# HKUST-Aerial-Robotics/D2SLAM

Measured on AMD Instinct MI355X. Metric: frames/sec SuperPoint+NetVLAD+match, 640x480 stereo, higher is better.
Workload: dtype f32

## Files before the change

### d2slam_amd/api.py

```python
import ctypes as C
import os
from dataclasses import dataclass, field
from typing import List, Optional

import numpy as np

from .weights import SP_LAYERS

_HERE = os.path.dirname(os.path.abspath(__file__))
LIB_PATH = os.path.join(_HERE, "lib", "libd2fe_hip.so")
DEV_LIB_PATH = os.path.join(_HERE, "lib", "libd2fe_hip_dev.so")
if os.environ.get("D2FE_LIB"):
    LIB_PATH = os.path.abspath(os.environ["D2FE_LIB"])

POSTPROC_B, POSTPROC_A = 0, 1
PREC_F32, PREC_F16X2, PREC_F32_WINO = 0, 1, 2
ERR_TRUNCATED = -4
KEEP_ALL_CAP = 1024
PROF_STAGES = ["conv1a", "conv1b", "conv2a", "conv2b", "conv3a", "conv3b", "conv4a", "conv4b", "convPaDa",
               "convPb", "convDb", "softmax_cand", "select", "sample", "match", "netvlad", "lk"]


class D2FEError(RuntimeError):
    def __init__(self, code, msg):
# ... 186 lines not shown
    "d2fe_quad_pipe_lanes", "d2fe_quad_pipe_geometry", "d2fe_quad_undistort_device",
    "d2fe_quad_device_view", "d2fe_quad_device_release", "d2fe_quad_lane_stream", "d2fe_quad_handle",
    "d2fe_quad_exchange_default_config", "d2fe_quad_exchange_create", "d2fe_quad_exchange_destroy", "d2fe_quad_exchange_enqueue", "d2fe_quad_exchange_collect",
    "d2fe_quad_exchange_jobs", "d2fe_quad_exchange_pairs", "d2fe_quad_exchange_block_bytes", "d2fe_quad_exchange_stream", "d2fe_quad_exchange_gathered", "d2fe_quad_exchange_job_layout",
    "d2fe_exchange_default_config", "d2fe_exchange_create", "d2fe_exchange_destroy", "d2fe_exchange_enqueue", "d2fe_exchange_collect", "d2fe_exchange_pairs",
    "d2fe_exchange_block_bytes", "d2fe_exchange_stream", "d2fe_exchange_gathered",
    "d2fe_window_default_config", "d2fe_window_create", "d2fe_window_create_quad", "d2fe_window_destroy", "d2fe_window_stream", "d2fe_window_push",
    "d2fe_window_push_host", "d2fe_window_retain", "d2fe_window_retain_plan", "d2fe_window_size", "d2fe_window_tags", "d2fe_window_track_device", "d2fe_window_collect",
    "d2fe_loop_default_config", "d2fe_loop_create", "d2fe_loop_create_quad", "d2fe_loop_destroy", "d2fe_loop_enqueue", "d2fe_loop_collect", "d2fe_loop_ntotal",
    "d2fe_loop_keyframes", "d2fe_loop_stream", "d2fe_loop_query_device", "d2fe_loop_add_host", "d2fe_rccl_load", "d2fe_rccl_path", "d2fe_rccl_unique_id", "d2fe_rccl_comm_init_rank", "d2fe_rccl_comm_destroy"]
DEBUG_EXPORTS = [
    "d2fe_debug_graph_count", "d2fe_debug_read", "d2fe_debug_netvlad_layer", "d2fe_debug_netvlad_stamps", "d2fe_debug_pack_wino",
    "d2fe_debug_pack_netvlad", "d2fe_debug_netvlad_tile", "d2fe_debug_conv3x3_wino", "d2fe_debug_match_stamps",
    "d2fe_debug_netvlad_plan", "d2fe_debug_regime_counts", "d2fe_debug_regime_reset"]
REGIMES = ["wino_nt1_one", "wino_nt1_static", "wino_nt1_claimed", "wino_nt2_one", "wino_nt2_static", "wino_nt2_claimed_ring", "wino_nt2_claimed_fused1b",
           "match_nw4", "match_nw2", "nv_gmerge", "nv_front_tpw", "wino_last_grid", "wino_last_total"]


def _preload_hip_runtime():
    import importlib.util
    import sys
    if "torch" in sys.modules:
        return
    try:
        spec = importlib.util.find_spec("torch")
    except (ImportError, ValueError):
        spec = None
    if spec is not None and spec.origin:
        cand = os.path.join(os.path.dirname(spec.origin), "lib", "libamdhip64.so")
        if os.path.exists(cand):
            try:
# ... 1572 lines not shown
```

### d2slam_amd/build.py

```python
import json
import os
import subprocess
import sys
from concurrent.futures import ThreadPoolExecutor

HERE = os.path.dirname(os.path.abspath(__file__))
CSRC = os.path.join(HERE, "csrc")
LIBDIR = os.path.join(HERE, "lib")
LIB = os.path.join(LIBDIR, "libd2fe_hip.so")
SOURCES = ["api.hip", "conv.hip", "conv_f16.hip", "conv_pc.hip", "conv_wino.hip", "conv1x1.hip", "postproc.hip", "match.hip", "netvlad.hip", "netvlad_fused.hip", "netvlad_pair.hip", "netvlad_host.hip", "next.hip", "swarm.hip", "lk.hip", "lk_carry.hip", "pipe.hip", "exchange.hip", "quad_pipe.hip", "quad_exchange.hip", "loop.hip", "window.hip"]
HEADERS = ["kernels.h", "conv_common.h", "context.h", "stream_deal.h", "lk_device.h", "consumer.h", "lane_ring.h", "exchange_wire.h", os.path.join("..", "..", "include", "d2fe.h"), os.path.join("..", "..", "include", "d2fe_debug.h")]
FLAGS = ["--offload-arch=gfx950", "-O3", "-std=c++17", "-fPIC", "-ffp-contract=off", "-fvisibility=hidden",
         "-Wall", "-Wno-unused-function", "-Wno-unused-result", "-Wno-unused-value"]


EXTRA_FLAGS = {"conv_wino.hip": ["-mllvm", "-amdgpu-atomic-optimizer-strategy=None"]}


def _hipcc():
    for c in (os.environ.get("HIPCC"), "/opt/rocm/bin/hipcc", "hipcc"):
        if c and (os.path.isabs(c) and os.path.exists(c) or not os.path.isabs(c)):
            return c
    return "hipcc"


def needs_build(lib=None):
# ... 78 lines not shown
```

### d2slam_amd/csrc/api.hip

```cpp
#include <hip/hip_runtime.h>

#include <algorithm>
#include <cmath>
#include <cstdio>
#include <cstring>
#include <cstdlib>
#include <array>
#include <atomic>
#include <deque>
#include <map>
#include <mutex>
#include <string>
#include <vector>

#include "context.h"
#ifdef D2FE_DEVTOOLS
#include "../../include/d2fe_debug.h"
#endif

using namespace d2fe;

namespace {
thread_local std::string g_err;
}
// ... 81 lines not shown
    return fail(D2FE_ERR_INVALID, std::string("superpoint layer ") + name + ": unexpected shape");
  return D2FE_OK;
}

}

namespace d2fe {
void graphs_clear(d2fe_context* h) {
  if (h->graphs.empty()) return;
  (void)hipStreamSynchronize(h->stream);
  for (auto& kv : h->graphs) if (kv.second.exec) (void)hipGraphExecDestroy(kv.second.exec);
  h->graphs.clear();
}

void host_state_save(const d2fe_context* h, d2fe_context::HostState& st) {
  st.last_w = h->last_w; st.last_h = h->last_h; st.last_n = h->last_n; st.last_set = h->last_set;
  st.last_gray = h->last_gray; st.last_stride = h->last_stride; st.last_istride = h->last_istride;
  st.nv = h->nv_run.last;
}
void host_state_restore(d2fe_context* h, const d2fe_context::HostState& st, bool netvlad) {
  if (netvlad) {
    h->nv_run.last = st.nv;
  } else {
    h->last_w = st.last_w; h->last_h = st.last_h; h->last_n = st.last_n; h->last_set = st.last_set;
    h->last_gray = st.last_gray; h->last_stride = st.last_stride; h->last_istride = st.last_istride;
  }
}

int run_superpoint(d2fe_context* h, const uint8_t* d_gray, int n, int W, int H, int stride, size_t image_stride,
                   float* d_kps, float* d_scores, float* d_desc, int32_t* d_idx, int cap, int32_t* d_n, hipStream_t s,
                   hipStream_t s_tail, int bs) {
  Tensor& a4b = bs ? h->a4b2 : h->a4b;
  Tensor& logits = bs ? h->logits2 : h->logits;
  Tensor& draw = bs ? h->draw2 : h->draw;
  h->last_set = bs;
  const int prec = h->cfg.precision;
  const bool tail_elsewhere = s_tail && s_tail != s;
  const bool wctr = prec == D2FE_PREC_F32_WINO && h->wino_dynamic;
  if (wctr || !tail_elsewhere)
// ... 7 lines not shown
    a.cout_real = L.cout; a.wpack = L.wpack; a.bias = L.bias;
    a.img = d_gray; a.img_stride = stride; a.img_istride = (long)image_stride; a.w1a = h->w1a; a.b1a = h->b1a;
    a.H = hh; a.W = ww; a.n_img = n; a.in_img_stride = iis; a.out_img_stride = ois; a.zeros = h->zeros; a.ncu = h->ncu;
    a.tag = (&L == &h->L[L_1B]) ? 1 : 0;
    a.work_ctr = (prec == D2FE_PREC_F32_WINO && h->wino_dynamic) ? h->work_ctrs + (int)(&L - &h->L[0]) : nullptr;
    { static const int ab = d2fe_dev_env("D2FE_ABLATE", 0); a.ablate = ab; }
    if (prec != D2FE_PREC_F16X2 && shape == CONV_256_1x1_T4x16 && L.cout == 65 && !pool && !relu) {
      static const int on = d2fe_dev_env("D2FE_CONV1X1", 1);
      if (on) { const hipError_t e = launch_conv1x1_256_65(a, s); if (e != hipErrorNotSupported) return e; }
    }
    if (prec == D2FE_PREC_F32_WINO)
      return shape == CONV1B_FUSED ? launch_conv_wino_fused1b(L.cout_pad, a, s)
             : (L.ks == 3 && !direct) ? launch_conv_wino(L.cin, pool, relu, L.cout_pad, a, s) : launch_conv(shape, D2FE_PREC_F32, pool, relu, L.cout_pad, a, s);
    return launch_conv(shape, prec, pool, relu, L.cout_pad, a, s);
  };
  if (h->fuse1a) {
    ProfScope ps(h, D2FE_PROF_CONV1B, s);
    HIP_TRY(conv(CONV1B_FUSED, h->L[L_1B], nullptr, 64, 0, 0, h->a1b.p, 64, (long)H2 * W2 * 64, H, W, true, true));
  } else {
    { ProfScope ps(h, D2FE_PROF_CONV1A, s); HIP_TRY(launch_conv1a(d_gray, stride, (long)image_stride, H, W, n, h->w1a, h->b1a, h->a1a.p, s)); }
    { ProfScope ps(h, D2FE_PROF_CONV1B, s); HIP_TRY(conv(CONV_64_T8x32, h->L[L_1B], h->a1a.p, 64, 0, (long)H * W * 64, h->a1b.p, 64, (long)H2 * W2 * 64, H, W, true, true)); }
  }
  { ProfScope ps(h, D2FE_PROF_CONV2A, s); HIP_TRY(conv(CONV_64_T8x32, h->L[L_2A], h->a1b.p, 64, 0, (long)H2 * W2 * 64, h->a2a.p, 64, (long)H2 * W2 * 64, H2, W2, false, true)); }
  { ProfScope ps(h, D2FE_PROF_CONV2B, s); HIP_TRY(conv(CONV_64_T8x32, h->L[L_2B], h->a2a.p, 64, 0, (long)H2 * W2 * 64, h->a2b.p, 64, (long)H4 * W4 * 64, H2, W2, true, true)); }
  { ProfScope ps(h, D2FE_PROF_CONV3A, s); HIP_TRY(conv(CONV_64_T8x32, h->L[L_3A], h->a2b.p, 64, 0, (long)H4 * W4 * 64, h->a3a.p, 128, (long)H4 * W4 * 128, H4, W4, false, true)); }
  { ProfScope ps(h, D2FE_PROF_CONV3B, s); HIP_TRY(conv(CONV_128_T4x32, h->L[L_3B], h->a3a.p, 128, 0, (long)H4 * W4 * 128, h->a3b.p, 128, (long)Hc * Wc * 128, H4, W4, true, true)); }
  { ProfScope ps(h, D2FE_PROF_CONV4A, s); HIP_TRY(conv(CONV_128_T4x16, h->L[L_4A], h->a3b.p, 128, 0, (long)Hc * Wc * 128, h->a4a.p, 128, (long)Hc * Wc * 128, Hc, Wc, false, true)); }
  { ProfScope ps(h, D2FE_PROF_CONV4B, s); HIP_TRY(conv(CONV_128_T4x16, h->L[L_4B], h->a4a.p, 128, 0, (long)Hc * Wc * 128, a4b.p, 128, (long)Hc * Wc * 128, Hc, Wc, false, true)); }
  const bool sparse = h->sparse_desc && n >= h->sp_min_batch && 4 * (long)cap <= h->sp_slots;
  if (sparse) {
    { ProfScope ps(h, D2FE_PROF_CONVPADA, s); HIP_TRY(conv(CONV_128_T4x16, h->L[L_PA], a4b.p, 128, 0, (long)Hc * Wc * 128, h->aPD.p, 256, (long)Hc * Wc * 256, Hc, Wc, false, true)); }
    { ProfScope ps(h, D2FE_PROF_CONVPB, s); HIP_TRY(conv(CONV_256_1x1_T4x16, h->L[L_PB], h->aPD.p, 256, 0, (long)Hc * Wc * 256, logits.p, 65, (long)Hc * Wc * 65, Hc, Wc, false, false)); }
  } else {
    if (prec == D2FE_PREC_F32_WINO && h->sparse_desc) {
      ProfScope ps(h, D2FE_PROF_CONVPADA, s);
      HIP_TRY(conv(CONV_128_T4x16, h->L[L_PA], a4b.p, 128, 0, (long)Hc * Wc * 128, h->aPD.p, 512, (long)Hc * Wc * 512, Hc, Wc, false, true));
      HIP_TRY(conv(CONV_128_T4x16, h->L[L_DA32], a4b.p, 128, 0, (long)Hc * Wc * 128, h->aPD.p, 512, (long)Hc * Wc * 512, Hc, Wc, false, true, 256, true));
    } else
    { ProfScope ps(h, D2FE_PROF_CONVPADA, s); HIP_TRY(conv(CONV_128_T4x16, h->L[L_PADA], a4b.p, 128, 0, (long)Hc * Wc * 128, h->aPD.p, 512, (long)Hc * Wc * 512, Hc, Wc, false, true)); }
    { ProfScope ps(h, D2FE_PROF_CONVPB, s); HIP_TRY(conv(CONV_256_1x1_T4x16, h->L[L_PB], h->aPD.p, 512, 0, (long)Hc * Wc * 512, logits.p, 65, (long)Hc * Wc * 65, Hc, Wc, false, false)); }
    { ProfScope ps(h, D2FE_PROF_CONVDB, s); HIP_TRY(conv(CONV_256_1x1_T4x16, h->L[L_DB], h->aPD.p, 512, 256, (long)Hc * Wc * 512, draw.p, 256, (long)Hc * Wc * 256, Hc, Wc, false, false)); }
  }
  const bool varA = h->cfg.postproc == D2FE_POSTPROC_A;
  if (s_tail && s_tail != s) {
    HIP_TRY(hipEventRecord(h->ev_trunk[bs], s));
    HIP_TRY(hipStreamWaitEvent(s_tail, h->ev_trunk[bs], 0));
    s = s_tail;
  }
  { ProfScope ps(h, D2FE_PROF_SOFTMAX, s);
  HIP_TRY(launch_softmax_cand(logits.p, 65, Hc, Wc, n, h->cfg.keypoint_threshold, h->cfg.remove_borders,
                              (h->cfg.keep_score_map || varA || h->cfg.max_keypoints < 0) ? h->semi.p : nullptr,
                              h->cand, h->cand_count, varA ? 0 : h->cand_cap, tail_elsewhere, s)); }
  if (varA) {
    ProfScope ps(h, D2FE_PROF_SELECT, s);
    HIP_TRY(launch_nms2_a(h->semi.p, H, W, n, h->cfg.keypoint_threshold, h->cfg.nms_dist, h->aconf, h->clist, h->cand,
                          h->cand_count, h->cand_cap, h->a_ncand, s));
    HIP_TRY(launch_select_b(h->cand, h->cand_count, h->cand_cap, n, W, h->cfg.max_keypoints < 0 ? h->a_scap : h->cfg.max_keypoints, cap, 1, nullptr, H,
                            h->cfg.keypoint_threshold, 0, d_kps, d_scores, d_idx, d_n, s));
    if ((long)H * W > 65536)
      HIP_TRY(launch_nms2_wrap_fix(h->clist, h->a_ncand, H, W, n, d_kps, d_idx, d_n, cap, s));
  } else {
    ProfScope ps(h, D2FE_PROF_SELECT, s);
    HIP_TRY(launch_select_b(h->cand, h->cand_count, h->cand_cap, n, Wc * 8, h->cfg.max_keypoints, cap, 0,
                            (h->cfg.keep_score_map || h->cfg.max_keypoints < 0) ? h->semi.p : nullptr, Hc * 8, h->cfg.keypoint_threshold,
                            h->cfg.remove_borders, d_kps, d_scores, d_idx, d_n, s));
  }
  if (!sparse) {
// ... 3 lines not shown
                              h->pca_mean, h->pca_dims, h->a_samp, h->a_scap, h->a_cn, nullptr, 0, d_desc, s));
    else
      HIP_TRY(launch_sample_b(draw.p, 256, 0, Hc, Wc, n, d_kps, d_n, cap, nullptr, 0, d_desc, s));
  } else {
    { ProfScope ps(h, D2FE_PROF_CONVDB, s);
      HIP_TRY(launch_desc_head_sparse(d_kps, d_n, cap, Hc, Wc, n, a4b.p, 128, (long)Hc * Wc * 128, h->L[L_DA32].wpack, h->L[L_DA32].bias,
                                      h->L[L_DB32].wpack, h->L[L_DB32].bias, h->sp_flags, h->sp_slotmap, h->sp_cells, h->sp_count,
                                      h->sp_slots, h->sp_desc, h->sp_mid, h->sp_mid_imgs, varA ? W : 0, varA ? H : 0, s)); }
    ProfScope ps(h, D2FE_PROF_SAMPLE, s);
    if (varA)
      HIP_TRY(launch_sample_a(h->sp_desc, 256, 0, Hc, Wc, W, H, n, d_kps, d_n, cap, h->pca_dims ? h->pca_comp_t : nullptr,
                              h->pca_mean, h->pca_dims, h->a_samp, h->a_scap, h->a_cn, h->sp_slotmap, h->sp_slots, d_desc, s));
    else
      HIP_TRY(launch_sample_b(h->sp_desc, 256, 0, Hc, Wc, n, d_kps, d_n, cap, h->sp_slotmap, h->sp_slots, d_desc, s));
  }
  h->last_w = W; h->last_h = H; h->last_n = n;
  h->last_gray = d_gray; h->last_stride = stride; h->last_istride = image_stride;
  return D2FE_OK;
}

int check_geometry(d2fe_context* h, int n, int W, int H, int stride, int cap) {
  if (!h) return fail(D2FE_ERR_INVALID, "null handle");
  if (!h->sp_loaded) return fail(D2FE_ERR_NOT_READY, "superpoint weights not loaded");
  if (n < 1 || n > h->cfg.max_batch) return fail(D2FE_ERR_INVALID, "batch size out of range");
  if (W < 16 || H < 16 || W > h->cfg.max_width || H > h->cfg.max_height || (long)W * H > (long)h->cfg.max_width * h->cfg.max_height)
    return fail(D2FE_ERR_INVALID, "image size must be at least 16x16 and within the configured maximum");
  if (((W | H) & 7) && h->cfg.postproc == D2FE_POSTPROC_A)
    return fail(D2FE_ERR_INVALID, "post-processing variant A needs image sizes that are multiples of 8");
  if (stride < W) return fail(D2FE_ERR_INVALID, "stride < width");
  if (cap < 1) return fail(D2FE_ERR_INVALID, "cap < 1");
  return D2FE_OK;
// ... 50 lines not shown
    int rc = 0;
    if (!h->fuse1a) rc |= alloc_f(h->a1a, H * W * 64, B);
    rc |= alloc_f(h->a1b, H * W * 16, B);
    rc |= alloc_f(h->a2a, H * W * 16, B);
    rc |= alloc_f(h->a2b, H * W * 4, B);
    rc |= alloc_f(h->a3a, H * W * 8, B);
    rc |= alloc_f(h->a3b, H * W * 2, B);
    rc |= alloc_f(h->a4a, H * W * 2, B);
    rc |= alloc_f(h->a4b, H * W * 2, B);
    rc |= alloc_f(h->aPD, H * W * 8, B);
    rc |= alloc_f(h->logits, (H / 8) * (W / 8) * 65, B);
    rc |= alloc_f(h->draw, H * W * 4, B);
    rc |= alloc_f(h->semi, H * W, B);
    if (rc) return D2FE_ERR_HIP;
    h->cand_cap = (long)(H * W);
    HIP_TRY(hipMalloc(&h->cand, sizeof(unsigned long long) * h->cand_cap * B));
    HIP_TRY(hipMalloc(&h->work_ctrs, (64 + ((size_t)B + 63) / 64 * 64) * sizeof(int)));
    HIP_TRY(hipMemset(h->work_ctrs, 0, (64 + ((size_t)B + 63) / 64 * 64) * sizeof(int)));
    h->cand_count = h->work_ctrs + 64;
    if (cfg->async_tail) {
      HIP_TRY(hipStreamCreateWithFlags(&h->tail_stream, hipStreamNonBlocking));
      for (int i = 0; i < 2; ++i) {
        HIP_TRY(hipEventCreateWithFlags(&h->ev_trunk[i], hipEventDisableTiming));
        HIP_TRY(hipEventCreateWithFlags(&h->ev_tail[i], hipEventDisableTiming));
      }
      if (alloc_f(h->a4b2, H * W * 2, B) || alloc_f(h->logits2, (H / 8) * (W / 8) * 65, B) || alloc_f(h->draw2, H * W * 4, B)) return D2FE_ERR_HIP;
    }
    h->sparse_desc = !cfg->dense_descriptors;
    if (cfg->precision == D2FE_PREC_F32_WINO) h->sp_min_batch = 2;
    h->sp_min_batch = d2fe_dev_env("D2FE_SPARSE_MIN_BATCH", h->sp_min_batch);
// ... 891 lines not shown
long d2fe_debug_read(d2fe_handle h, const char* name, void* dst, size_t max_bytes) {
  if (!h || !name || !dst) return fail(D2FE_ERR_INVALID, "null argument");
  if (h->last_n == 0) return fail(D2FE_ERR_NOT_READY, "no extract call yet");
  hipSetDevice(h->cfg.device_id);
  const size_t H = h->last_h, W = h->last_w, n = h->last_n;
  struct { const char* nm; Tensor* t; size_t per; } tab[] = {
      {"conv1a", &h->a1a, H * W * 64},           {"conv1b", &h->a1b, (H / 2) * (W / 2) * 64},   {"conv2a", &h->a2a, (H / 2) * (W / 2) * 64},
      {"conv2b", &h->a2b, (H / 4) * (W / 4) * 64},   {"conv3a", &h->a3a, (H / 4) * (W / 4) * 128},  {"conv3b", &h->a3b, (H / 8) * (W / 8) * 128},
      {"conv4a", &h->a4a, (H / 8) * (W / 8) * 128},  {"conv4b", h->last_set ? &h->a4b2 : &h->a4b, (H / 8) * (W / 8) * 128},  {"convPaDa", &h->aPD, (H / 8) * (W / 8) * 512},
      {"logits", h->last_set ? &h->logits2 : &h->logits, (H / 8) * (W / 8) * 65}, {"desc_raw", h->last_set ? &h->draw2 : &h->draw, (H / 8) * (W / 8) * 256}, {"semi", &h->semi, (H / 8) * (W / 8) * 64}};
  if (!strcmp(name, "conv1a") && h->fuse1a) {
    if (!h->a1a.p && alloc_f(h->a1a, (size_t)h->cfg.max_height * h->cfg.max_width * 64, h->cfg.max_batch) != 0)
      return fail(D2FE_ERR_HIP, "hipMalloc conv1a debug buffer");
    if (launch_conv1a(h->last_gray, h->last_stride, (long)h->last_istride, (int)H, (int)W, (int)n, h->w1a, h->b1a, h->a1a.p, h->stream) != hipSuccess)
      return fail(D2FE_ERR_HIP, "conv1a debug launch");
  }
  if (!strcmp(name, "semi") && !h->cfg.keep_score_map) return fail(D2FE_ERR_NOT_READY, "score map not kept (set keep_score_map)");
  if (h->sparse_desc && h->last_n >= h->sp_min_batch && (!strcmp(name, "desc_raw") || !strcmp(name, "convPaDa")))
    return fail(D2FE_ERR_NOT_READY, "the dense descriptor map does not exist with the sparse descriptor head (set dense_descriptors)");
  for (auto& e : tab)
    if (!strcmp(e.nm, name)) {
      const size_t bytes = e.per * n * sizeof(float);
      if (bytes > max_bytes) return fail(D2FE_ERR_TRUNCATED, "destination too small");
      if (hipStreamSynchronize(h->stream) != hipSuccess || (h->tail_stream && hipStreamSynchronize(h->tail_stream) != hipSuccess)) return fail(D2FE_ERR_HIP, "sync");
      if (hipMemcpy(dst, e.t->p, bytes, hipMemcpyDeviceToHost) != hipSuccess) return fail(D2FE_ERR_HIP, "D2H");
      return (long)bytes;
    }
  return fail(D2FE_ERR_INVALID, "unknown tensor name");
}

// ... 175 lines not shown
```

### d2slam_amd/csrc/context.h

```cpp
#pragma once
#include <hip/hip_runtime.h>

#include <atomic>

#include <array>
#include <deque>
#include <map>
#include <memory>
#include <mutex>
#include <string>
#include <vector>

#include "../../include/d2fe.h"
#include "kernels.h"

namespace d2fe {
int ctx_fail(int code, const std::string& msg);
}

#define HIP_TRY(expr)                                                                                       \
  do {                                                                                                      \
    hipError_t e_ = (expr);                                                                                 \
    if (e_ != hipSuccess)                                                                                   \
      return d2fe::ctx_fail(D2FE_ERR_HIP, std::string(#expr) + ": " + hipGetErrorString(e_) + " @" + __FILE__ + ":" + \
// ... 81 lines not shown
  std::atomic<int> live_pipes{0};
  float* w1a = nullptr;
  float* b1a = nullptr;
  d2fe::Layer L[d2fe::L_COUNT];
  d2fe::Tensor a1a, a1b, a2a, a2b, a3a, a3b, a4a, a4b, aPD, logits, draw, semi;
  d2fe::Tensor a4b2, logits2, draw2;
  hipStream_t tail_stream = nullptr;
  hipEvent_t ev_trunk[2] = {nullptr, nullptr}, ev_tail[2] = {nullptr, nullptr};
  int parity = 0, last_set = 0;
  unsigned long long* cand = nullptr;
  int* cand_count = nullptr;
  long cand_cap = 0;
  uint8_t* s_img = nullptr;
  int s_cap = 0;
  int last_w = 0, last_h = 0, last_n = 0;
  const uint8_t* last_gray = nullptr; int last_stride = 0; size_t last_istride = 0;
  float* aconf = nullptr; int* clist = nullptr; int* a_ncand = nullptr;
  float* zeros = nullptr;
  uint8_t* pin_in = nullptr; size_t pin_in_bytes = 0;
  float* pin_out = nullptr; size_t pin_out_bytes = 0;
  float* s_out = nullptr;
  size_t s_out_bytes = 0;
  bool use_graphs = true, use_pinned = true;
  hipStream_t nv_stream = nullptr; hipEvent_t ev_up = nullptr; float* pin_nv = nullptr; size_t pin_nv_bytes = 0;
  struct HostState { int last_w = 0, last_h = 0, last_n = 0, last_set = 0; const uint8_t* last_gray = nullptr; int last_stride = 0; size_t last_istride = 0;
                     d2fe::NvLast nv; };
  struct GraphEntry { hipGraphExec_t exec = nullptr; int seen = 0; bool bad = false; HostState st; };
  std::map<std::array<long, 6>, GraphEntry> graphs;
  int ncu = 256;
  int ncu_dev = 256;
  unsigned long long* match_stamps = nullptr;
  int32_t* match_stats = nullptr;
  int* work_ctrs = nullptr;
  bool wino_dynamic = true;
  bool sparse_desc = false; int sp_slots = 0; int sp_min_batch = 4;
  uint8_t* sp_flags = nullptr; int32_t* sp_slotmap = nullptr; int32_t* sp_cells = nullptr; int32_t* sp_count = nullptr; float* sp_desc = nullptr;
  float* sp_mid = nullptr; int sp_mid_imgs = 0;
  void* lk_scratch = nullptr; size_t lk_scratch_bytes = 0;
  float* a_samp = nullptr; float* a_cn = nullptr; int a_scap = 0;
  float* pca_comp_t = nullptr; float* pca_mean = nullptr; int pca_dims = 0;
// ... 85 lines not shown
```

### d2slam_amd/csrc/conv1x1.hip

```cpp
#include "conv_common.h"

namespace d2fe {

namespace {
constexpr int C1_CIN = 256, C1_C8 = C1_CIN / 8, C1_RING = 8;
}

__global__ __launch_bounds__(256, 2) void conv1x1_256_65_kernel(ConvArgs a, long npix) {
  extern __shared__ __attribute__((aligned(16))) float wsm[];
  const int tid = threadIdx.x, lane = tid & 63, wave = tid >> 6, hh = lane >> 5;
  const float* wp = reinterpret_cast<const float*>(a.wpack);
  for (int i = tid; i < 2 * C1_C8 * 64; i += 256)
    reinterpret_cast<f32x4*>(wsm)[i] = reinterpret_cast<const f32x4*>(wp)[i];
  float* wdl = wsm + 2 * C1_C8 * 256;
  if (tid < C1_C8 * 8) {
    const int g = tid >> 3, h = (tid >> 2) & 1, q = tid & 3;
    wdl[tid] = wp[((size_t)2 * C1_C8 + g) * 256 + h * 128 + q];
  }
  const float bias0 = a.bias[lane & 31], bias1 = a.bias[32 + (lane & 31)], biasd = a.bias[64];
  __syncthreads();

  const long n_mt = (npix + 31) / 32;
  const int ics = a.in_cstride, ocs = a.out_cstride;
  for (long mt = (long)blockIdx.x * 4 + wave; mt < n_mt; mt += (long)gridDim.x * 4) {
// ... 55 lines not shown
  const long hw = (long)a.H * a.W;
  if (a.cout_real != 65 || a.in_img_stride != hw * a.in_cstride || a.out_img_stride != hw * a.out_cstride || a.out_cstride < 65 ||
      (a.in_cstride & 3) || (a.in_coff & 3) || a.in_coff + 256 > a.in_cstride)
    return hipErrorNotSupported;
  const int ncu = a.ncu > 0 ? a.ncu : 256;
  const long npix = hw * a.n_img;
  const long n_wg = (npix + 127) / 128;
  const int grid = (int)(n_wg < 2 * ncu ? n_wg : 2 * ncu);
  constexpr size_t lds = (size_t)(2 * C1_C8 * 256 + C1_C8 * 8) * sizeof(float);
  hipError_t e = hipFuncSetAttribute(reinterpret_cast<const void*>(conv1x1_256_65_kernel), hipFuncAttributeMaxDynamicSharedMemorySize, (int)lds);
  if (e != hipSuccess) return e;
  hipLaunchKernelGGL(conv1x1_256_65_kernel, dim3(grid), dim3(256), lds, s, a, npix);
  return hipGetLastError();
}

}
```

### d2slam_amd/csrc/kernels.h

```cpp
#pragma once
#include <hip/hip_runtime.h>
#include <stdint.h>

#ifdef D2FE_DEVTOOLS
#include <cstdlib>
static inline int d2fe_dev_env(const char* name, int dflt) { const char* e = getenv(name); return e ? atoi(e) : dflt; }
#define D2FE_ABL(a, bits) ((a).ablate & (bits))
#define D2FE_STAMP(buf, wg, i) do { if ((buf) && threadIdx.x == 0) (buf)[(size_t)(wg) * 16 + (i)] = wall_clock64(); } while (0)
#else
static inline int d2fe_dev_env(const char*, int dflt) { return dflt; }
#define D2FE_ABL(a, bits) (0)
#define D2FE_STAMP(buf, wg, i) do {} while (0)
#endif

#ifdef D2FE_DEVTOOLS
#include "../../include/d2fe_debug.h"
namespace d2fe { void regime_note(int regime); void regime_set(int regime, long long value); }
#define D2FE_REGIME(r) ::d2fe::regime_note(r)
#define D2FE_REGIME_SET(r, v) ::d2fe::regime_set(r, v)
#else
#define D2FE_REGIME(r) do {} while (0)
#define D2FE_REGIME_SET(r, v) do {} while (0)
#endif

// ... 19 lines not shown
  int ncu = 0;
};

enum ConvShape {
  CONV_64_T8x32 = 0,
  CONV_128_T4x32,
  CONV_128_T4x16,
  CONV_256_1x1_T4x16,
  CONV1B_FUSED,
};

hipError_t launch_conv(ConvShape shape, int precision, bool pool, bool relu, int cout_pad, const ConvArgs& a,
                       hipStream_t s);

hipError_t launch_conv1x1_256_65(const ConvArgs& a, hipStream_t s);

hipError_t launch_conv_pc(ConvShape shape, int precision, bool pool, bool relu, int cout_pad, const ConvArgs& a, hipStream_t s);

hipError_t launch_conv_wino(int cin, bool pool, bool relu, int cout_pad, const ConvArgs& a, hipStream_t s);
hipError_t launch_conv_wino_fused1b(int cout_pad, const ConvArgs& a, hipStream_t s);
size_t packed_weight_floats_wino(int cout_pad, int cin);
void pack_weights_wino(const float* w , int cout, int cin, int cout_pad, float* dst);

hipError_t launch_conv1a(const uint8_t* img, int stride, long img_stride_bytes, int H, int W, int n,
                         const float* w9x64 , const float* bias, float* out, hipStream_t s);

size_t packed_weight_floats_f32(int cout_pad, int cin, int ks);
void pack_weights_f32(const float* w , int cout, int cin, int ks, int cout_pad, float* dst);
size_t packed_weight_halfs_f16x2(int cout_pad, int cin, int ks);
void pack_weights_f16x2(const float* w, int cout, int cin, int ks, int cout_pad, uint16_t* dst);
// ... 145 lines not shown
```

### d2slam_amd/csrc/postproc.hip

```cpp
#include <algorithm>

#include "kernels.h"

namespace d2fe {

typedef float f32x4 __attribute__((ext_vector_type(4)));
typedef float f32x16 __attribute__((ext_vector_type(16)));

__device__ __forceinline__ float d2fe_expf(float x) {
  if (x < -87.0f) x = -87.0f;
  const float t = x * 1.44269504088896341f;
  const float n = __builtin_rintf(t);
  float r = __builtin_fmaf(n, -0.693359375f, x);
  r = __builtin_fmaf(n, 2.12194440e-4f, r);
  float p = 1.9875691500E-4f;
  p = __builtin_fmaf(p, r, 1.3981999507E-3f);
  p = __builtin_fmaf(p, r, 8.3334519073E-3f);
  p = __builtin_fmaf(p, r, 4.1665795894E-2f);
  p = __builtin_fmaf(p, r, 1.6666665459E-1f);
  p = __builtin_fmaf(p, r, 5.0000001201E-1f);
  const float r2 = r * r;
  const float y = __builtin_fmaf(p, r2, r) + 1.0f;
  return __builtin_ldexpf(y, (int)n);
}

__global__ __launch_bounds__(256) void softmax_cand_kernel(const float* __restrict__ logits, int lstride, int Hc, int Wc,
                                                           float thr, int border, float* __restrict__ semi,
                                                           unsigned long long* __restrict__ cand,
                                                           int* __restrict__ cand_count, long cand_cap) {
  __shared__ float sl[64 * 65];
  const int img = blockIdx.y;
  const int ncell = Hc * Wc;
  const int cell0 = blockIdx.x * 64;
  const int tid = threadIdx.x, lane = tid & 63;
  const float* lg = logits + ((size_t)img * ncell + cell0) * lstride;
  const int nvalid = min(64, ncell - cell0);
  if (lstride == 65) {
    for (int i = tid; i < nvalid * 65; i += 256) sl[i] = lg[i];
  } else {
// ... 828 lines not shown
```

### include/d2fe_debug.h

```cpp
#ifndef D2FE_DEBUG_H_
#define D2FE_DEBUG_H_

#include "d2fe.h"

#ifdef __cplusplus
extern "C" {
#endif

D2FE_API long d2fe_debug_read(d2fe_handle h, const char* name, void* dst, size_t max_bytes);
D2FE_API long d2fe_debug_netvlad_layer(d2fe_handle h, int layer, int n_images, void* dst, size_t max_bytes);
D2FE_API long d2fe_debug_netvlad_stamps(d2fe_handle h, unsigned long long* dst, long max_wgs);
D2FE_API int d2fe_debug_netvlad_plan(const d2fe_nv_layer* layers, int n_layers, int proj_dim, int* out, int max_steps);
D2FE_API int d2fe_debug_netvlad_tile(int kind, int Ho, int Wo, int stride, int* th, int* tw);
D2FE_API long d2fe_debug_pack_netvlad(int kind, const float* we, const float* be, const float* wd, const float* bd, const float* wp, int cin, int chid,
                                      int cout, float* out, long max_floats);
D2FE_API long d2fe_debug_pack_wino(const float* weight , int cout, int cin, float* out, long max_floats);
D2FE_API int d2fe_debug_conv3x3_wino(d2fe_handle h, const float* in, int n, int H, int W, int cin, const float* weight,
                                     const float* bias, int cout, int pool, int relu, float* out, int iters, float* ms_per_launch);

D2FE_API int d2fe_debug_graph_count(d2fe_handle h, int* rejected);

enum d2fe_regime {
  D2FE_REGIME_WINO_NT1_ONE = 0,
  D2FE_REGIME_WINO_NT1_STATIC,
  D2FE_REGIME_WINO_NT1_CLAIMED,
  D2FE_REGIME_WINO_NT2_ONE,
  D2FE_REGIME_WINO_NT2_STATIC,
  D2FE_REGIME_WINO_NT2_CLAIMED_RING,
  D2FE_REGIME_WINO_NT2_CLAIMED_FUSED1B,
  D2FE_REGIME_MATCH_NW4,
  D2FE_REGIME_MATCH_NW2,
  D2FE_REGIME_NV_GMERGE,
  D2FE_REGIME_NV_FRONT_TPW,
  D2FE_REGIME_WINO_LAST_GRID,
  D2FE_REGIME_WINO_LAST_TOTAL,
  D2FE_REGIME_COUNT
};
D2FE_API int d2fe_debug_regime_counts(long long* out, int max);
D2FE_API void d2fe_debug_regime_reset(void);

D2FE_API long d2fe_debug_match_stamps(d2fe_handle h, unsigned long long* dst, long max_wgs);

#ifdef __cplusplus
}
#endif
#endif
```

Measured before the change: 2336.

## Fuse detector head 1x1 conv with softmax and candidate extraction

Adds a single kernel that computes the 256->65 convPb 1x1 conv with MFMA, then applies the 65-way softmax and threshold/border test and appends keypoint candidates directly. It runs when score maps are not needed, replacing the conv + softmax_cand kernel pair. This avoids writing and re-reading the logits buffer and saves one launch. In exchange it adds a complex persistent kernel with wave-level atomics for the candidate append, and a debug path that recomputes logits on demand.

Result: no change. 2340 (median of 2 runs) (+0.1%).

```diff
diff --git a/d2slam_amd/api.py b/d2slam_amd/api.py
--- a/d2slam_amd/api.py
+++ b/d2slam_amd/api.py
@@ -224,7 +224,7 @@
     "d2fe_debug_pack_netvlad", "d2fe_debug_netvlad_tile", "d2fe_debug_conv3x3_wino", "d2fe_debug_match_stamps",
     "d2fe_debug_netvlad_plan", "d2fe_debug_regime_counts", "d2fe_debug_regime_reset"]
 REGIMES = ["wino_nt1_one", "wino_nt1_static", "wino_nt1_claimed", "wino_nt2_one", "wino_nt2_static", "wino_nt2_claimed_ring", "wino_nt2_claimed_fused1b",
-           "match_nw4", "match_nw2", "nv_gmerge", "nv_front_tpw", "wino_last_grid", "wino_last_total"]
+           "match_nw4", "match_nw2", "nv_gmerge", "nv_front_tpw", "head_fused", "wino_last_grid", "wino_last_total"]
 
 
 def _preload_hip_runtime():
diff --git a/d2slam_amd/build.py b/d2slam_amd/build.py
--- a/d2slam_amd/build.py
+++ b/d2slam_amd/build.py
@@ -9,7 +9,7 @@
 LIBDIR = os.path.join(HERE, "lib")
 LIB = os.path.join(LIBDIR, "libd2fe_hip.so")
 SOURCES = ["api.hip", "conv.hip", "conv_f16.hip", "conv_pc.hip", "conv_wino.hip", "conv1x1.hip", "postproc.hip", "match.hip", "netvlad.hip", "netvlad_fused.hip", "netvlad_pair.hip", "netvlad_host.hip", "next.hip", "swarm.hip", "lk.hip", "lk_carry.hip", "pipe.hip", "exchange.hip", "quad_pipe.hip", "quad_exchange.hip", "loop.hip", "window.hip"]
-HEADERS = ["kernels.h", "conv_common.h", "context.h", "stream_deal.h", "lk_device.h", "consumer.h", "lane_ring.h", "exchange_wire.h", os.path.join("..", "..", "include", "d2fe.h"), os.path.join("..", "..", "include", "d2fe_debug.h")]
+HEADERS = ["kernels.h", "conv_common.h", "score_math.h", "context.h", "stream_deal.h", "lk_device.h", "consumer.h", "lane_ring.h", "exchange_wire.h", os.path.join("..", "..", "include", "d2fe.h"), os.path.join("..", "..", "include", "d2fe_debug.h")]
 FLAGS = ["--offload-arch=gfx950", "-O3", "-std=c++17", "-fPIC", "-ffp-contract=off", "-fvisibility=hidden",
          "-Wall", "-Wno-unused-function", "-Wno-unused-result", "-Wno-unused-value"]
 
diff --git a/d2slam_amd/csrc/api.hip b/d2slam_amd/csrc/api.hip
--- a/d2slam_amd/csrc/api.hip
+++ b/d2slam_amd/csrc/api.hip
@@ -119,7 +119,7 @@
 }
 
 void host_state_save(const d2fe_context* h, d2fe_context::HostState& st) {
-  st.last_w = h->last_w; st.last_h = h->last_h; st.last_n = h->last_n; st.last_set = h->last_set;
+  st.last_w = h->last_w; st.last_h = h->last_h; st.last_n = h->last_n; st.last_set = h->last_set; st.last_pd_stride = h->last_pd_stride;
   st.last_gray = h->last_gray; st.last_stride = h->last_stride; st.last_istride = h->last_istride;
   st.nv = h->nv_run.last;
 }
@@ -127,7 +127,7 @@
   if (netvlad) {
     h->nv_run.last = st.nv;
   } else {
-    h->last_w = st.last_w; h->last_h = st.last_h; h->last_n = st.last_n; h->last_set = st.last_set;
+    h->last_w = st.last_w; h->last_h = st.last_h; h->last_n = st.last_n; h->last_set = st.last_set; h->last_pd_stride = st.last_pd_stride;
     h->last_gray = st.last_gray; h->last_stride = st.last_stride; h->last_istride = st.last_istride;
   }
 }
@@ -165,6 +165,24 @@
              : (L.ks == 3 && !direct) ? launch_conv_wino(L.cin, pool, relu, L.cout_pad, a, s) : launch_conv(shape, D2FE_PREC_F32, pool, relu, L.cout_pad, a, s);
     return launch_conv(shape, prec, pool, relu, L.cout_pad, a, s);
   };
+  const bool varA = h->cfg.postproc == D2FE_POSTPROC_A;
+  const bool want_maps = h->cfg.keep_score_map || varA || h->cfg.max_keypoints < 0;
+  bool head_fused = false;
+  auto conv_pb = [&](int ics) -> int {
+    ProfScope ps(h, D2FE_PROF_CONVPB, s);
+    if (prec != D2FE_PREC_F16X2 && !tail_elsewhere && !want_maps && d2fe_dev_env("D2FE_HEAD_FUSED", 1)) {
+      ConvArgs a{};
+      a.in = h->aPD.p; a.in_cstride = ics; a.in_img_stride = (long)Hc * Wc * ics;
+      a.cout_real = h->L[L_PB].cout; a.wpack = h->L[L_PB].wpack; a.bias = h->L[L_PB].bias;
+      a.H = Hc; a.W = Wc; a.n_img = n; a.ncu = h->ncu;
+      const HeadArgs t{h->cfg.keypoint_threshold, h->cfg.remove_borders, h->cand, h->cand_count, h->cand_cap};
+      const hipError_t e = launch_detector_head_fused(a, t, s);
+      if (e == hipSuccess) { head_fused = true; D2FE_REGIME(D2FE_REGIME_HEAD_FUSED); return D2FE_OK; }
+      if (e != hipErrorNotSupported) HIP_TRY(e);
+    }
+    HIP_TRY(conv(CONV_256_1x1_T4x16, h->L[L_PB], h->aPD.p, ics, 0, (long)Hc * Wc * ics, logits.p, 65, (long)Hc * Wc * 65, Hc, Wc, false, false));
+    return D2FE_OK;
+  };
   if (h->fuse1a) {
     ProfScope ps(h, D2FE_PROF_CONV1B, s);
     HIP_TRY(conv(CONV1B_FUSED, h->L[L_1B], nullptr, 64, 0, 0, h->a1b.p, 64, (long)H2 * W2 * 64, H, W, true, true));
@@ -181,7 +199,7 @@
   const bool sparse = h->sparse_desc && n >= h->sp_min_batch && 4 * (long)cap <= h->sp_slots;
   if (sparse) {
     { ProfScope ps(h, D2FE_PROF_CONVPADA, s); HIP_TRY(conv(CONV_128_T4x16, h->L[L_PA], a4b.p, 128, 0, (long)Hc * Wc * 128, h->aPD.p, 256, (long)Hc * Wc * 256, Hc, Wc, false, true)); }
-    { ProfScope ps(h, D2FE_PROF_CONVPB, s); HIP_TRY(conv(CONV_256_1x1_T4x16, h->L[L_PB], h->aPD.p, 256, 0, (long)Hc * Wc * 256, logits.p, 65, (long)Hc * Wc * 65, Hc, Wc, false, false)); }
+    if (const int rc = conv_pb(256)) return rc;
   } else {
     if (prec == D2FE_PREC_F32_WINO && h->sparse_desc) {
       ProfScope ps(h, D2FE_PROF_CONVPADA, s);
@@ -189,19 +207,19 @@
       HIP_TRY(conv(CONV_128_T4x16, h->L[L_DA32], a4b.p, 128, 0, (long)Hc * Wc * 128, h->aPD.p, 512, (long)Hc * Wc * 512, Hc, Wc, false, true, 256, true));
     } else
     { ProfScope ps(h, D2FE_PROF_CONVPADA, s); HIP_TRY(conv(CONV_128_T4x16, h->L[L_PADA], a4b.p, 128, 0, (long)Hc * Wc * 128, h->aPD.p, 512, (long)Hc * Wc * 512, Hc, Wc, false, true)); }
-    { ProfScope ps(h, D2FE_PROF_CONVPB, s); HIP_TRY(conv(CONV_256_1x1_T4x16, h->L[L_PB], h->aPD.p, 512, 0, (long)Hc * Wc * 512, logits.p, 65, (long)Hc * Wc * 65, Hc, Wc, false, false)); }
+    if (const int rc = conv_pb(512)) return rc;
     { ProfScope ps(h, D2FE_PROF_CONVDB, s); HIP_TRY(conv(CONV_256_1x1_T4x16, h->L[L_DB], h->aPD.p, 512, 256, (long)Hc * Wc * 512, draw.p, 256, (long)Hc * Wc * 256, Hc, Wc, false, false)); }
   }
-  const bool varA = h->cfg.postproc == D2FE_POSTPROC_A;
   if (s_tail && s_tail != s) {
     HIP_TRY(hipEventRecord(h->ev_trunk[bs], s));
     HIP_TRY(hipStreamWaitEvent(s_tail, h->ev_trunk[bs], 0));
     s = s_tail;
   }
-  { ProfScope ps(h, D2FE_PROF_SOFTMAX, s);
-  HIP_TRY(launch_softmax_cand(logits.p, 65, Hc, Wc, n, h->cfg.keypoint_threshold, h->cfg.remove_borders,
-                              (h->cfg.keep_score_map || varA || h->cfg.max_keypoints < 0) ? h->semi.p : nullptr,
-                              h->cand, h->cand_count, varA ? 0 : h->cand_cap, tail_elsewhere, s)); }
+  if (!head_fused) {
+    ProfScope ps(h, D2FE_PROF_SOFTMAX, s);
+    HIP_TRY(launch_softmax_cand(logits.p, 65, Hc, Wc, n, h->cfg.keypoint_threshold, h->cfg.remove_borders, want_maps ? h->semi.p : nullptr,
+                                h->cand, h->cand_count, varA ? 0 : h->cand_cap, tail_elsewhere, s));
+  }
   if (varA) {
     ProfScope ps(h, D2FE_PROF_SELECT, s);
     HIP_TRY(launch_nms2_a(h->semi.p, H, W, n, h->cfg.keypoint_threshold, h->cfg.nms_dist, h->aconf, h->clist, h->cand,
@@ -235,7 +253,7 @@
     else
       HIP_TRY(launch_sample_b(h->sp_desc, 256, 0, Hc, Wc, n, d_kps, d_n, cap, h->sp_slotmap, h->sp_slots, d_desc, s));
   }
-  h->last_w = W; h->last_h = H; h->last_n = n;
+  h->last_w = W; h->last_h = H; h->last_n = n; h->last_pd_stride = head_fused ? (sparse ? 256 : 512) : 0;
   h->last_gray = d_gray; h->last_stride = stride; h->last_istride = image_stride;
   return D2FE_OK;
 }
@@ -316,6 +334,7 @@
     rc |= alloc_f(h->semi, H * W, B);
     if (rc) return D2FE_ERR_HIP;
     h->cand_cap = (long)(H * W);
+    { const int c = d2fe_dev_env("D2FE_CAND_CAP", 0); if (c > 0 && c < h->cand_cap) h->cand_cap = c; }
     HIP_TRY(hipMalloc(&h->cand, sizeof(unsigned long long) * h->cand_cap * B));
     HIP_TRY(hipMalloc(&h->work_ctrs, (64 + ((size_t)B + 63) / 64 * 64) * sizeof(int)));
     HIP_TRY(hipMemset(h->work_ctrs, 0, (64 + ((size_t)B + 63) / 64 * 64) * sizeof(int)));
@@ -1237,6 +1256,34 @@
       return fail(D2FE_ERR_HIP, "hipMalloc conv1a debug buffer");
     if (launch_conv1a(h->last_gray, h->last_stride, (long)h->last_istride, (int)H, (int)W, (int)n, h->w1a, h->b1a, h->a1a.p, h->stream) != hipSuccess)
       return fail(D2FE_ERR_HIP, "conv1a debug launch");
+  }
+  if (!strcmp(name, "logits") && h->last_pd_stride) {
+    ConvArgs a{};
+    const int ics = h->last_pd_stride, Hc = (int)(H / 8), Wc = (int)(W / 8);
+    a.in = h->aPD.p; a.in_cstride = ics; a.in_img_stride = (long)Hc * Wc * ics;
+    a.out = (h->last_set ? h->logits2 : h->logits).p; a.out_cstride = 65; a.out_img_stride = (long)Hc * Wc * 65;
+    a.cout_real = h->L[L_PB].cout; a.wpack = h->L[L_PB].wpack; a.bias = h->L[L_PB].bias;
+    a.H = Hc; a.W = Wc; a.n_img = (int)n; a.ncu = h->ncu;
+    if (launch_conv1x1_256_65(a, h->stream) != hipSuccess) return fail(D2FE_ERR_HIP, "convPb debug launch");
+  }
+  if (!strcmp(name, "cand_count") || !strcmp(name, "cand")) {
+    const bool keys = !strcmp(name, "cand");
+    if (hipStreamSynchronize(h->stream) != hipSuccess || (h->tail_stream && hipStreamSynchronize(h->tail_stream) != hipSuccess)) return fail(D2FE_ERR_HIP, "sync");
+    std::vector<int> cnt(n);
+    if (hipMemcpy(cnt.data(), h->cand_count, n * sizeof(int), hipMemcpyDeviceToHost) != hipSuccess) return fail(D2FE_ERR_HIP, "D2H");
+    if (!keys) {
+      if (n * sizeof(int) > max_bytes) return fail(D2FE_ERR_TRUNCATED, "destination too small");
+      memcpy(dst, cnt.data(), n * sizeof(int));
+      return (long)(n * sizeof(int));
+    }
+    const size_t per = max_bytes / n / sizeof(unsigned long long);
+    for (size_t i = 0; i < n; ++i) {
+      const size_t k = std::min<size_t>((size_t)std::max(cnt[i], 0), (size_t)h->cand_cap);
+      if (k > per) return fail(D2FE_ERR_TRUNCATED, "destination too small");
+      if (k && hipMemcpy(static_cast<unsigned long long*>(dst) + i * per, h->cand + i * (size_t)h->cand_cap, k * sizeof(unsigned long long), hipMemcpyDeviceToHost) != hipSuccess)
+        return fail(D2FE_ERR_HIP, "D2H");
+    }
+    return (long)max_bytes;
   }
   if (!strcmp(name, "semi") && !h->cfg.keep_score_map) return fail(D2FE_ERR_NOT_READY, "score map not kept (set keep_score_map)");
   if (h->sparse_desc && h->last_n >= h->sp_min_batch && (!strcmp(name, "desc_raw") || !strcmp(name, "convPaDa")))
diff --git a/d2slam_amd/csrc/context.h b/d2slam_amd/csrc/context.h
--- a/d2slam_amd/csrc/context.h
+++ b/d2slam_amd/csrc/context.h
@@ -119,6 +119,7 @@
   uint8_t* s_img = nullptr;
   int s_cap = 0;
   int last_w = 0, last_h = 0, last_n = 0;
+  int last_pd_stride = 0;
   const uint8_t* last_gray = nullptr; int last_stride = 0; size_t last_istride = 0;
   float* aconf = nullptr; int* clist = nullptr; int* a_ncand = nullptr;
   float* zeros = nullptr;
@@ -128,7 +129,7 @@
   size_t s_out_bytes = 0;
   bool use_graphs = true, use_pinned = true;
   hipStream_t nv_stream = nullptr; hipEvent_t ev_up = nullptr; float* pin_nv = nullptr; size_t pin_nv_bytes = 0;
-  struct HostState { int last_w = 0, last_h = 0, last_n = 0, last_set = 0; const uint8_t* last_gray = nullptr; int last_stride = 0; size_t last_istride = 0;
+  struct HostState { int last_w = 0, last_h = 0, last_n = 0, last_set = 0, last_pd_stride = 0; const uint8_t* last_gray = nullptr; int last_stride = 0; size_t last_istride = 0;
                      d2fe::NvLast nv; };
   struct GraphEntry { hipGraphExec_t exec = nullptr; int seen = 0; bool bad = false; HostState st; };
   std::map<std::array<long, 6>, GraphEntry> graphs;
diff --git a/d2slam_amd/csrc/conv1x1.hip b/d2slam_amd/csrc/conv1x1.hip
--- a/d2slam_amd/csrc/conv1x1.hip
+++ b/d2slam_amd/csrc/conv1x1.hip
@@ -1,4 +1,5 @@
 #include "conv_common.h"
+#include "score_math.h"
 
 namespace d2fe {
 
@@ -93,4 +94,203 @@
   return hipGetLastError();
 }
 
-}
+namespace {
+constexpr int FH_WAVES = 8;
+constexpr int FH_SC = 32, FH_NS = C1_CIN / FH_SC;
+constexpr int FH_ROW = FH_SC + 4;
+constexpr int FH_BUF = 32 * FH_ROW;
+constexpr int FH_WAVE = 2 * FH_BUF;
+constexpr int FH_TP = 65;
+static_assert(32 * FH_TP + 1 <= FH_WAVE, "the transposed logits overlay the slice buffers");
+constexpr int FH_WFLOATS = 2 * C1_C8 * 256 + C1_C8 * 8;
+constexpr size_t FH_LDS = (size_t)(FH_WFLOATS + FH_WAVES * FH_WAVE) * sizeof(float);
+}
+
+__global__ __launch_bounds__(64 * FH_WAVES) void detector_head_fused_kernel(ConvArgs a, long npix, HeadArgs t) {
+  extern __shared__ __attribute__((aligned(16))) float wsm[];
+  const int tid = threadIdx.x, lane = tid & 63, wave = tid >> 6, hh = lane >> 5, li = lane & 31;
+  const float* wp = reinterpret_cast<const float*>(a.wpack);
+  for (int i = tid; i < 2 * C1_C8 * 64; i += 64 * FH_WAVES)
+    reinterpret_cast<f32x4*>(wsm)[i] = reinterpret_cast<const f32x4*>(wp)[i];
+  float* wdl = wsm + 2 * C1_C8 * 256;
+  if (tid < C1_C8 * 8) {
+    const int g = tid >> 3, h = (tid >> 2) & 1, q = tid & 3;
+    wdl[tid] = wp[((size_t)2 * C1_C8 + g) * 256 + h * 128 + q];
+  }
+  const float bias0 = a.bias[li], bias1 = a.bias[32 + li], biasd = a.bias[64];
+  __syncthreads();
+  if (wave < 4) __builtin_amdgcn_s_setprio(1);
+
+  float* ring = wsm + FH_WFLOATS + wave * FH_WAVE;
+  const long n_mt = (npix + 31) / 32;
+  const long step = (long)gridDim.x * FH_WAVES;
+  long mt = (long)wave * gridDim.x + blockIdx.x;
+  if (mt >= n_mt) return;
+  const int ics = a.in_cstride;
+  const int srow = lane >> 3, sch = (lane & 7) * 4;
+  const float* in = a.in + a.in_coff + sch;
+  size_t so[4], sn[4];
+#pragma unroll
+  for (int j = 0; j < 4; ++j) {
+    const long p = mt * 32 + j * 8 + srow;
+    so[j] = (size_t)(p < npix ? p : npix - 1) * ics;
+  }
+  f32x4 R[2][4];
+#pragma unroll
+  for (int j = 0; j < 4; ++j) {
+    R[0][j] = *reinterpret_cast<const f32x4*>(in + so[j]);
+    R[1][j] = *reinterpret_cast<const f32x4*>(in + so[j] + FH_SC);
+  }
+  const unsigned ncell = (unsigned)a.H * (unsigned)a.W;
+  const int Wc = a.W, W = a.W * 8, H = a.H * 8;
+#pragma unroll 1
+  for (; mt < n_mt; mt += step) {
+    const long nxt = mt + step < n_mt ? mt + step : mt;
+#pragma unroll
+    for (int j = 0; j < 4; ++j) {
+      const long p = nxt * 32 + j * 8 + srow;
+      sn[j] = (size_t)(p < npix ? p : npix - 1) * ics;
+    }
+    f32x16 acc0, acc1;
+#pragma unroll
+    for (int r = 0; r < 16; ++r) { acc0[r] = bias0; acc1[r] = bias1; }
+    float d = biasd;
+#pragma unroll
+    for (int s = 0; s < FH_NS; ++s) {
+      float* buf = ring + (s & 1) * FH_BUF;
+      wave_lds_order();
+#pragma unroll
+      for (int j = 0; j < 4; ++j) *reinterpret_cast<f32x4*>(buf + (j * 8 + srow) * FH_ROW + sch) = R[s & 1][j];
+#pragma unroll
+      for (int j = 0; j < 4; ++j)
+        R[s & 1][j] = *reinterpret_cast<const f32x4*>(in + (s + 2 < FH_NS ? so[j] + (s + 2) * FH_SC : sn[j] + (s + 2 - FH_NS) * FH_SC));
+      wave_lds_order();
+#pragma unroll
+      for (int gg = 0; gg < FH_SC / 8; ++gg) {
+        const int g = s * (FH_SC / 8) + gg;
+        const f32x4 x0 = *reinterpret_cast<const f32x4*>(buf + li * FH_ROW + gg * 8);
+        const f32x4 x1 = *reinterpret_cast<const f32x4*>(buf + li * FH_ROW + gg * 8 + 4);
+        const f32x4 b0 = reinterpret_cast<const f32x4*>(wsm)[(0 * C1_C8 + g) * 64 + lane];
+        const f32x4 b1 = reinterpret_cast<const f32x4*>(wsm)[(1 * C1_C8 + g) * 64 + lane];
+        const float a0 = hh ? x0[1] : x0[0], a1 = hh ? x0[3] : x0[2], a2 = hh ? x1[1] : x1[0], a3 = hh ? x1[3] : x1[2];
+        acc0 = __builtin_amdgcn_mfma_f32_32x32x2f32(a0, b0[0], acc0, 0, 0, 0);
+        acc1 = __builtin_amdgcn_mfma_f32_32x32x2f32(a0, b1[0], acc1, 0, 0, 0);
+        acc0 = __builtin_amdgcn_mfma_f32_32x32x2f32(a1, b0[1], acc0, 0, 0, 0);
+        acc1 = __builtin_amdgcn_mfma_f32_32x32x2f32(a1, b1[1], acc1, 0, 0, 0);
+        acc0 = __builtin_amdgcn_mfma_f32_32x32x2f32(a2, b0[2], acc0, 0, 0, 0);
+        acc1 = __builtin_amdgcn_mfma_f32_32x32x2f32(a2, b1[2], acc1, 0, 0, 0);
+        acc0 = __builtin_amdgcn_mfma_f32_32x32x2f32(a3, b0[3], acc0, 0, 0, 0);
+        acc1 = __builtin_amdgcn_mfma_f32_32x32x2f32(a3, b1[3], acc1, 0, 0, 0);
+        const f32x4 we = reinterpret_cast<const f32x4*>(wdl)[g * 2], wo = reinterpret_cast<const f32x4*>(wdl)[g * 2 + 1];
+        d = __builtin_fmaf(x0[0], we[0], d);   d = __builtin_fmaf(x0[1], wo[0], d);
+        d = __builtin_fmaf(x0[2], we[1], d);   d = __builtin_fmaf(x0[3], wo[1], d);
+        d = __builtin_fmaf(x1[0], we[2], d);   d = __builtin_fmaf(x1[1], wo[2], d);
+        d = __builtin_fmaf(x1[2], we[3], d);   d = __builtin_fmaf(x1[3], wo[3], d);
+      }
+    }
+#pragma unroll
+    for (int j = 0; j < 4; ++j) so[j] = sn[j];
+
+    float* T = ring;
+    wave_lds_order();
+#pragma unroll
+    for (int r = 0; r < 16; ++r) {
+      const int pl = (r & 3) + 8 * (r >> 2) + 4 * hh;
+      T[pl * FH_TP + li] = acc0[r];
+      T[pl * FH_TP + 32 + li] = acc1[r];
+    }
+    T[li * FH_TP + 64] = d;
+    wave_lds_order();
+    constexpr int NV = 33;
+    int c0 = hh ? 33 : 0;
+    asm volatile("" : "+v"(c0));
+    const int nc = hh ? 32 : 33;
+    const float* l = T + li * FH_TP + c0;
+    float v[NV];
+    float m = l[0];
+#pragma unroll
+    for (int k = 0; k < NV; ++k) {
+      v[k] = l[k < nc ? k : 0];
+      m = v[k] > m ? v[k] : m;
+    }
+    m = fmaxf(m, __shfl_xor(m, 32, 64));
+#pragma unroll
+    for (int k = 0; k < NV; ++k) v[k] = d2fe_expf(v[k] - m);
+    float sum = 0.f;
+#pragma unroll
+    for (int q = 0; q < 2; ++q) {
+      if (hh == q) {
+#pragma unroll
+        for (int k = 0; k < NV; ++k)
+          if (k < nc) sum += v[k];
+      }
+      sum = __shfl(sum, li + 32 * q, 64);
+    }
+    const long pg = mt * 32 + li;
+    const bool live = pg < npix;
+    const unsigned pu = live ? (unsigned)pg : 0u;
+    const int img = (int)(pu / ncell);
+    const int cell = (int)(pu - (unsigned)img * ncell);
+    const int cy = cell / Wc, cx = cell - cy * Wc;
+    int mine = 0;
+    unsigned long long pass = 0;
+#pragma unroll
+    for (int k = 0; k < NV; ++k) {
+      const int c = c0 + k;
+      if (c < 64) {
+        const float p = v[k] / sum;
+        v[k] = p;
+        const int y = cy * 8 + (c >> 3), x = cx * 8 + (c & 7);
+        if (live && p > t.thr && y >= t.border && y < H - t.border && x >= t.border && x < W - t.border) { ++mine; pass |= 1ull << k; }
+      }
+    }
+    int slot = 0;
+    unsigned long long todo = __ballot(mine > 0);
+    while (todo) {
+      const int img0 = __shfl(img, __ffsll((long long)todo) - 1, 64);
+      const bool in = mine > 0 && img == img0;
+      const int cnt = in ? mine : 0;
+      int incl = cnt;
+#pragma unroll
+      for (int o = 1; o < 64; o <<= 1) {
+        const int u = __shfl_up(incl, o, 64);
+        if (lane >= o) incl += u;
+      }
+      const int total = __shfl(incl, 63, 64);
+      int base = 0;
+      if (lane == 0) base = atomicAdd(t.cand_count + img0, total);
+      base = __shfl(base, 0, 64);
+      if (in) slot = base + incl - cnt;
+      todo &= ~__ballot(in);
+    }
+    unsigned long long* cd = t.cand + (size_t)img * t.cand_cap;
+#pragma unroll
+    for (int k = 0; k < NV; ++k) {
+      if (pass & (1ull << k)) {
+        const int c = c0 + k;
+        const int y = cy * 8 + (c >> 3), x = cx * 8 + (c & 7);
+        const unsigned idx = (unsigned)(y * W + x);
+        if (slot < t.cand_cap)
+          cd[slot] = ((unsigned long long)__float_as_uint(v[k]) << 32) | (unsigned long long)(0xFFFFFFFFu - idx);
+        ++slot;
+      }
+    }
+  }
+}
+
+hipError_t launch_detector_head_fused(const ConvArgs& a, const HeadArgs& t, hipStream_t s) {
+  const long hw = (long)a.H * a.W;
+  const long npix = hw * a.n_img;
+  if (a.cout_real != 65 || a.in_img_stride != hw * a.in_cstride || (a.in_cstride & 3) || (a.in_coff & 3) || a.in_coff + 256 > a.in_cstride ||
+      npix < 1 || npix >= (1l << 31) || !t.cand || !t.cand_count)
+    return hipErrorNotSupported;
+  const int ncu = a.ncu > 0 ? a.ncu : 256;
+  const long n_mt = (npix + 31) / 32;
+  const int grid = (int)(n_mt < ncu ? n_mt : ncu);
+  hipError_t e = hipFuncSetAttribute(reinterpret_cast<const void*>(detector_head_fused_kernel), hipFuncAttributeMaxDynamicSharedMemorySize, (int)FH_LDS);
+  if (e != hipSuccess) return e;
+  hipLaunchKernelGGL(detector_head_fused_kernel, dim3(grid), dim3(64 * FH_WAVES), FH_LDS, s, a, npix, t);
+  return hipGetLastError();
+}
+
+}
diff --git a/d2slam_amd/csrc/kernels.h b/d2slam_amd/csrc/kernels.h
--- a/d2slam_amd/csrc/kernels.h
+++ b/d2slam_amd/csrc/kernels.h
@@ -57,6 +57,9 @@
                        hipStream_t s);
 
 hipError_t launch_conv1x1_256_65(const ConvArgs& a, hipStream_t s);
+
+struct HeadArgs { float thr; int border; unsigned long long* cand; int* cand_count; long cand_cap; };
+hipError_t launch_detector_head_fused(const ConvArgs& a, const HeadArgs& t, hipStream_t s);
 
 hipError_t launch_conv_pc(ConvShape shape, int precision, bool pool, bool relu, int cout_pad, const ConvArgs& a, hipStream_t s);
 
diff --git a/d2slam_amd/csrc/postproc.hip b/d2slam_amd/csrc/postproc.hip
--- a/d2slam_amd/csrc/postproc.hip
+++ b/d2slam_amd/csrc/postproc.hip
@@ -1,28 +1,12 @@
 #include <algorithm>
 
 #include "kernels.h"
+#include "score_math.h"
 
 namespace d2fe {
 
 typedef float f32x4 __attribute__((ext_vector_type(4)));
 typedef float f32x16 __attribute__((ext_vector_type(16)));
-
-__device__ __forceinline__ float d2fe_expf(float x) {
-  if (x < -87.0f) x = -87.0f;
-  const float t = x * 1.44269504088896341f;
-  const float n = __builtin_rintf(t);
-  float r = __builtin_fmaf(n, -0.693359375f, x);
-  r = __builtin_fmaf(n, 2.12194440e-4f, r);
-  float p = 1.9875691500E-4f;
-  p = __builtin_fmaf(p, r, 1.3981999507E-3f);
-  p = __builtin_fmaf(p, r, 8.3334519073E-3f);
-  p = __builtin_fmaf(p, r, 4.1665795894E-2f);
-  p = __builtin_fmaf(p, r, 1.6666665459E-1f);
-  p = __builtin_fmaf(p, r, 5.0000001201E-1f);
-  const float r2 = r * r;
-  const float y = __builtin_fmaf(p, r2, r) + 1.0f;
-  return __builtin_ldexpf(y, (int)n);
-}
 
 __global__ __launch_bounds__(256) void softmax_cand_kernel(const float* __restrict__ logits, int lstride, int Hc, int Wc,
                                                            float thr, int border, float* __restrict__ semi,
diff --git a/d2slam_amd/csrc/score_math.h b/d2slam_amd/csrc/score_math.h
--- /dev/null
+++ b/d2slam_amd/csrc/score_math.h
@@ -0,0 +1,29 @@
+#pragma once
+#include <hip/hip_runtime.h>
+
+namespace d2fe {
+
+__device__ __forceinline__ float d2fe_expf(float x) {
+  if (x < -87.0f) x = -87.0f;
+  const float t = x * 1.44269504088896341f;
+  const float n = __builtin_rintf(t);
+  float r = __builtin_fmaf(n, -0.693359375f, x);
+  r = __builtin_fmaf(n, 2.12194440e-4f, r);
+  float p = 1.9875691500E-4f;
+  p = __builtin_fmaf(p, r, 1.3981999507E-3f);
+  p = __builtin_fmaf(p, r, 8.3334519073E-3f);
+  p = __builtin_fmaf(p, r, 4.1665795894E-2f);
+  p = __builtin_fmaf(p, r, 1.6666665459E-1f);
+  p = __builtin_fmaf(p, r, 5.0000001201E-1f);
+  const float r2 = r * r;
+  const float y = __builtin_fmaf(p, r2, r) + 1.0f;
+  return __builtin_ldexpf(y, (int)n);
+}
+
+__device__ __forceinline__ void wave_lds_order() {
+  __builtin_amdgcn_fence(__ATOMIC_RELEASE, "wavefront");
+  __builtin_amdgcn_wave_barrier();
+  __builtin_amdgcn_fence(__ATOMIC_ACQUIRE, "wavefront");
+}
+
+}
diff --git a/include/d2fe_debug.h b/include/d2fe_debug.h
--- a/include/d2fe_debug.h
+++ b/include/d2fe_debug.h
@@ -32,6 +32,7 @@
   D2FE_REGIME_MATCH_NW2,
   D2FE_REGIME_NV_GMERGE,
   D2FE_REGIME_NV_FRONT_TPW,
+  D2FE_REGIME_HEAD_FUSED,
   D2FE_REGIME_WINO_LAST_GRID,
   D2FE_REGIME_WINO_LAST_TOTAL,
   D2FE_REGIME_COUNT
```
